# feiyuhuahuo/Yolact_minimal

Measured on AMD Instinct MI355X. Metric: img/s res101_coco 544x544 inference (bs=1/GPU, 4 requests in flight), higher is better.
Workload: dtype f32; 1 GPU; res101_coco 544x544 (the reference's "550-class" size) bs=1 inference: forward + nms + after_nms(480x640) per image, 4 independent bs=1 requests in flight on 4 HIP streams; global_batch=1, parallelism=replicas x1 (inference does not shard), weights=seeded random init, post_inputs=synthetic dense head outputs (17.8k candidates), requests_in_flight=4

## Files before the change

include/yolact_hip.h:

```cpp
#ifndef YOLACT_HIP_H
#define YOLACT_HIP_H

#include <stddef.h>
#include <stdint.h>

#ifdef __cplusplus
extern "C" {
#endif

#define YM_OK 0
#define YM_EINVAL (-1)
#define YM_ENOSPC (-2)
#define YM_ELAUNCH (-3)

#define YM_ACT_NONE 0
#define YM_ACT_RELU 1
#define YM_ACT_TANH 2
#define YM_ACT_GELU 3

typedef void* ym_stream_t;

int ym_abi_version(void);
const char* ym_last_error(void);

// ... 189 lines not shown
int ym_match_anchors_batch(const float* const* gt_boxes_cls, const int32_t* g, int B, const float* anchors, int N, float pos_thre,
                           float neg_thre, float* offsets, int64_t* conf, float* anchor_box, int64_t* anchor_gt, void* workspace,
                           size_t workspace_bytes, ym_stream_t s);

size_t ym_loss_workspace_bytes(int B, int N);
int ym_class_box_loss(const float* class_p, const float* box_p, const float* offsets, const int64_t* conf, int B, int N, int C,
                      float conf_alpha, float bbox_alpha, int neg_pos_ratio, float* dclass, float* dbox, int32_t* num_pos,
                      double* loss_c, double* loss_b, void* workspace, size_t workspace_bytes, ym_stream_t s);

int ym_select_positives(const int64_t* conf, const float* keys, int B, int N, int cap, const int32_t* num_pos, int64_t* idx,
                        ym_stream_t s);

int ym_gt_masks_downsample(const float* masks, int n, int H, int W, int out_h, int out_w, float* out, ym_stream_t s);

int ym_semantic_loss(const float* seg_nhwc, int P, int pitch, int num_classes, const float* gt_masks_ds, const int64_t* gt_cls,
                     int gt_cls_stride, int g, float coeff, float* dseg, double* loss_accum, ym_stream_t s);
int ym_semantic_loss_batch(const float* seg_nhwc, int B, int P, int pitch, int num_classes, const float* const* gt_masks_ds,
                           const int64_t* const* gt_cls, int gt_cls_stride, const int32_t* g, float coeff, float* dseg,
                           double* loss_accum, ym_stream_t s);

int ym_maxpool3x3s2_bwd(const float* x, const float* dy, float* dx, int B, int H, int W, int C, ym_stream_t s);
int ym_maxpool3x3s2_fwd_idx(const float* in, float* out, uint8_t* idx, int B, int H, int W, int C, ym_stream_t s);
int ym_maxpool3x3s2_bwd_idx(const uint8_t* idx, const float* dy, float* dx, int B, int H, int W, int C, ym_stream_t s);
int ym_bilinear2x_bwd(const float* dy, float* dx, int B, int H, int W, int C, int align_corners, ym_stream_t s);

int ym_sgd_step(float* param, const float* grad, float* momentum_buf, int64_t n, float lr, float momentum,
                float weight_decay, int first_step, ym_stream_t s);


int ym_maxpool3x3s2_fwd(const float* in, float* out, int B, int H, int W, int C, ym_stream_t s);
int ym_stem_conv_bn_relu_maxpool(const float* img_nchw, const float* w_packed, const float* scale, const float* shift, float* out,
                                 int B, int H, int W, int k_pad, ym_stream_t s);

int ym_bilinear2x_fwd(const float* in, float* out, int B, int H, int W, int C, int align_corners, ym_stream_t s);

int ym_softmax_rows(const float* in, float* out, int64_t rows, int C, ym_stream_t s);


int ym_layernorm(const float* x, const float* gamma, const float* beta, float eps, float* out, int64_t M, int C,
                 ym_stream_t s);

int ym_patch_merge_layernorm(const float* x, int B, int H, int W, int C, const float* gamma, const float* beta, float eps,
                             float* out, ym_stream_t s);

int ym_swin_window_attention(const float* qkv, const float* qkv_bias, const float* rel_bias_table, int B, int H, int W, int C,
                             int heads, int window, int shift, float* out, ym_stream_t s);


int ym_val_preprocess(const void* img_hwc_bgr, int is_uint8, int H, int W, int S, const float* mean_bgr,
                      const float* std_bgr, float* out_chw_rgb, ym_stream_t s);


typedef struct {
    int32_t num_anchors;
    int32_t num_classes;
    int32_t coef_dim;
    int32_t top_k;
    int32_t max_det;
    float score_thre;
    float iou_thre;
    float img_size;
} ym_nms_cfg;

size_t ym_nms_workspace_bytes(const ym_nms_cfg* cfg);

int ym_detect_fast_nms(const float* class_pred, const float* box_pred, const float* coef_pred,
// ... 124 lines not shown
```

yolact_minimal_amd/engine.py:

```python
import json
import os
import sys

import torch
import torch.nn as nn

from . import conv_launch, hip, plan_transfer
from .conv_plan import ConvPlan
from .hip import ACT_NONE, ACT_RELU, ACT_TANH, ACT_GELU


def _round_up(x, m):
    return (x + m - 1) // m * m


TUNED_PATH = os.environ.get('YM_TUNED_PATH', os.path.join(os.path.dirname(os.path.abspath(__file__)), 'tuned_gfx950.json'))
_tuned = None


def conv_mma():
    return int(os.environ.get('YM_CONV_MMA', '0') or 0)


def no_tuned():
# ... 135 lines not shown
        self._bind_params()
        self.out_hw = (ho, wo)
        self.flops = 2.0 * b * ho * wo * self.cout * self.kh * self.kw * self.cin
        self.sig = plan_transfer.forward_key(b * ho * wo, self.cout, cin, self.kh, self.stride, len(segs), residual is not None)
        self._shape = (b * ho * wo, self.cout, self.k_pad // 32, len(segs))
        self._resolve(conv_mma())
        return ho, wo

    def _resolve(self, mma, bound=None, pyramid=False):
        d = self.desc
        self.plan, self.mma, self.plan_source, self._hit = conv_launch.infer_plan(
            tuned_table(), self.sig, self._shape, _build_mode[0], mma, not self.stem and d.Cin % 32 == 0 and d.nlevels == 0, self.plan,
            no_tuned(), pyramid, bound)
        self.plan.apply(d)
        d.mma = self.mma

    def apply_mma(self, mma):
        self._resolve(mma, (self._hit, self.plan_source))


def _bind_pyramid(layer, pyr, batch, shapes, segs):
    rows, cin = pyr.shape
    assert cin == layer.cin_pad and layer.stride == 1 and layer.pad == layer.kh // 2 and len(shapes) <= 5
    assert rows == sum(batch * h * w for h, w in shapes)
    d = layer.desc = conv_launch.conv_desc(batch, shapes[0][0], shapes[0][1], cin, layer.cout, layer.kh, layer.kw, 1, layer.pad,
                                           shapes[0][0], shapes[0][1], layer.k_pad, segs, levels=shapes)
    d.inp = pyr.data_ptr()
    layer._bind_params()
    layer.out_hw = shapes[0]
    layer.flops = 2.0 * rows * layer.cout * layer.kh * layer.kw * layer.cin
    layer.sig = plan_transfer.forward_key(rows, layer.cout, cin, layer.kh, 1, len(segs), levels=len(shapes))
    layer._shape = (rows, layer.cout, layer.k_pad // 32, len(segs))
    layer._resolve(0, pyramid=True)


class InferEngine:
    def __init__(self, net, batch, height, width, device, use_graph=None, mode='latency'):
        self.net = net
        self.mode = mode
        self.device = device
        self.B, self.H, self.W = batch, height, width
        self.num_classes = net.cfg.num_classes
        self.coef_dim = net.coef_dim
        self.na = len(net.cfg.aspect_ratios)
        if use_graph is None:
            use_graph = os.environ.get('YM_GRAPH', '1') != '0'
        self.use_graph = use_graph
        self.graph = None
        self.ops = []
        self.op_stream = {}
        self.op_deps = {}
        self._producers = {}
        self._cur_stream = 0
        self._side_streams = {}
        self._events = {}
        self.use_branches = os.environ.get('YM_BRANCHES', '0') == '1'
        self.convs = []
        self.fused_stem = None
        self._img = None
        self._weights_epoch = -1
        self._bufs = []
        hip.lib()
        prev, _build_mode[0] = _build_mode[0], mode
        try:
            with torch.cuda.device(device):
                self._build()
                if autotune_on() and not no_tuned():
                    self._autotune_missing()
        finally:
            _build_mode[0] = prev

    def _autotune_missing(self):
        have = {c.sig for c in self.convs if c.plan_source == 'table'}
        todo = {c.sig for c in self.convs} - have
        if not todo:
            return
        rows = self.autotune(iters=10, skip=have)
        for c in self.convs:
            if c.sig in rows:
                c.plan_source, c._hit = 'autotuned', ConvPlan.from_row(rows[c.sig])
        record_rows(rows)

    def _buf(self, *shape):
        t = torch.empty(*shape, device=self.device, dtype=torch.float32)
        self._bufs.append(t)
        return t

    def _add_op(self, kind, arg, inputs, outputs):
        idx = len(self.ops)
        self.ops.append((kind, arg))
        sid = self._cur_stream if self.use_branches else 0
        self.op_stream[idx] = sid
        deps = []
        for t in inputs:
            if t is None:
                continue
            for j in self._producers.get(t.data_ptr(), ()):
                if self.op_stream[j] != sid and j not in deps:
                    deps.append(j)
        if deps:
            self.op_deps[idx] = deps
        for t in outputs:
            self._producers.setdefault(t.data_ptr(), []).append(idx)
        return idx

    def _conv(self, layer, x, out=None, residual=None, segs=None, seg_outputs=None):
        b, h, w, _ = x.shape
        ho = (h + 2 * layer.pad - layer.kh) // layer.stride + 1
        wo = (w + 2 * layer.pad - layer.kw) // layer.stride + 1
        if segs is None:
            if out is None:
                out = self._buf(b, ho, wo, layer.cout)
            segs = [(0, layer.cout, out.data_ptr(), ho * wo * layer.cout, layer.cout, layer.act)]
        layer.refresh()
        layer.bind(x, segs, residual)
        self.convs.append(layer)
        self._add_op('conv', layer, [x, residual], seg_outputs if seg_outputs is not None else [out])
        return out

    def _build_swin(self):
        net, B = self.net, self.B
        bb = net.backbone
        ws = bb.window_size
        assert self.H % 4 == 0 and self.W % 4 == 0
        pe = bb.patch_embed
        x = self._conv(_Conv('backbone.patch_embed.proj', pe.proj, act=ACT_NONE, stem=True), self.x_in)
        self._add_op('layernorm', (x, pe.norm, x), [x], [x])
        feats = []
        for li, layer in enumerate(bb.layers):
            _, h, w, c = x.shape
            heads = bb.heads[li]
            for bi, blk in enumerate(layer.blocks):
                p = f'backbone.layers.{li}.blocks.{bi}'
                n1 = self._buf(B, h, w, c)
                self._add_op('layernorm', (x, blk.norm1, n1), [x], [n1])
                qkv = self._conv(_Conv(p + '.attn.qkv', _LinearAsConv(blk.attn.qkv)), n1)
                att = self._buf(B, h, w, c)
                self._add_op('attn', (qkv, blk.attn, att, (B, h, w, c, heads, ws, blk.shift_size)), [qkv], [att])
                x = self._conv(_Conv(p + '.attn.proj', _LinearAsConv(blk.attn.proj)), att, residual=x)
                n2 = self._buf(B, h, w, c)
                self._add_op('layernorm', (x, blk.norm2, n2), [x], [n2])
                hid = self._conv(_Conv(p + '.mlp.fc1', _LinearAsConv(blk.mlp.fc1), act=ACT_GELU), n2)
                x = self._conv(_Conv(p + '.mlp.fc2', _LinearAsConv(blk.mlp.fc2)), hid, residual=x)
            if li in bb.out_norm_indices:
                f = self._buf(B, h, w, c)
                self._add_op('layernorm', (x, getattr(bb, f'norm{li}'), f), [x], [f])
                feats.append(f)
            if layer.downsample is not None:
                ho, wo = (h + 1) // 2, (w + 1) // 2
                merged = self._buf(B, ho, wo, 4 * c)
# ... 10 lines not shown
            c3, c4, c5 = self._build_swin()
        else:
            c3, c4, c5 = self._build_resnet()
        self._build_neck_and_heads(c3, c4, c5)

    def _build_resnet(self):
        net, B, H, W = self.net, self.B, self.H, self.W
        bb = net.backbone

        stem = _Conv('backbone.conv1', bb.conv1, bb.bn1, ACT_RELU, stem=True)
        conv1 = bb.conv1
        fusable = (conv1.out_channels == 64 and conv1.in_channels == 3 and tuple(conv1.kernel_size) == (7, 7) and
                   tuple(conv1.stride) == (2, 2) and tuple(conv1.padding) == (3, 3))
        if fusable and os.environ.get('YM_FUSED_STEM', '1') != '0':
            stem.refresh()
            ho, wo = (H + 6 - 7) // 2 + 1, (W + 6 - 7) // 2 + 1
            hp, wp = (ho + 2 - 3) // 2 + 1, (wo + 2 - 3) // 2 + 1
            stem.flops = 2.0 * B * ho * wo * stem.cout * stem.kh * stem.kw * stem.cin
            self.fused_stem = stem
            pooled = self._buf(B, hp, wp, 64)
            self._add_op('stem_pool', (stem, pooled), [], [pooled])
            x = pooled
        else:
            x = self._conv(stem, self.x_in)
            hp, wp = (x.shape[1] + 2 - 3) // 2 + 1, (x.shape[2] + 2 - 3) // 2 + 1
            pooled = self._buf(B, hp, wp, 64)
            self._add_op('maxpool', (x, pooled), [x], [pooled])
            x = pooled

        stage_outs = []
        for li, stage in enumerate(bb.layers):
            for bi, blk in enumerate(stage):
                p = f'backbone.layers.{li}.{bi}'
                y = self._conv(_Conv(p + '.conv1', blk.conv1, blk.bn1, ACT_RELU), x)
                y = self._conv(_Conv(p + '.conv2', blk.conv2, blk.bn2, ACT_RELU), y)
                if blk.downsample is not None:
                    skip = self._conv(_Conv(p + '.downsample', blk.downsample[0], blk.downsample[1], ACT_NONE), x)
                else:
                    skip = x
                x = self._conv(_Conv(p + '.conv3', blk.conv3, blk.bn3, ACT_RELU), y, residual=skip)
            stage_outs.append(x)
        return stage_outs[1:4]

    def _build_neck_and_heads(self, c3, c4, c5):
        net, B = self.net, self.B
        fpn = net.fpn
        p5_1 = self._conv(_Conv('fpn.lat_layers.2', fpn.lat_layers[2]), c5)
        u5 = self._buf(B, p5_1.shape[1] * 2, p5_1.shape[2] * 2, 256)
        self._add_op('bilinear', (p5_1, u5, False), [p5_1], [u5])
        assert u5.shape[1:3] == c4.shape[1:3], 'img_size must be divisible by 32 (reference config.py:75)'
        p4_1 = self._conv(_Conv('fpn.lat_layers.1', fpn.lat_layers[1]), c4, residual=u5)
        u4 = self._buf(B, p4_1.shape[1] * 2, p4_1.shape[2] * 2, 256)
        self._add_op('bilinear', (p4_1, u4, False), [p4_1], [u4])
        p3_1 = self._conv(_Conv('fpn.lat_layers.0', fpn.lat_layers[0]), c3, residual=u4)
        pyr_env = os.environ.get('YM_PYRAMID_HEAD', 'auto')
        pyramid = pyr_env == '1' or (pyr_env == 'auto' and B <= 2)
        h5, w5 = p5_1.shape[1:3]
        shapes = [tuple(p3_1.shape[1:3]), tuple(p4_1.shape[1:3]), (h5, w5), ((h5 + 1) // 2, (w5 + 1) // 2),
                  (((h5 + 1) // 2 + 1) // 2, ((w5 + 1) // 2 + 1) // 2)]
        rows = [B * h * w for h, w in shapes]
        pyr = self._buf(sum(rows), 256)
        views, r0 = [], 0
        for (h, w), n in zip(shapes, rows):
            views.append(pyr[r0:r0 + n].view(B, h, w, 256))
            r0 += n
        self._cur_stream = 1
        p5 = self._conv(_Conv('fpn.pred_layers.2', fpn.pred_layers[2][0], act=ACT_RELU), p5_1, out=views[2])
        p6 = self._conv(_Conv('fpn.downsample_layers.0', fpn.downsample_layers[0][0], act=ACT_RELU), p5, out=views[3])
        p7 = self._conv(_Conv('fpn.downsample_layers.1', fpn.downsample_layers[1][0], act=ACT_RELU), p6, out=views[4])
        self._cur_stream = 2
        p4 = self._conv(_Conv('fpn.pred_layers.1', fpn.pred_layers[1][0], act=ACT_RELU), p4_1, out=views[1])
        self._cur_stream = 0
        p3 = self._conv(_Conv('fpn.pred_layers.0', fpn.pred_layers[0][0], act=ACT_RELU), p3_1, out=views[0])
# ... 37 lines not shown
            self.convs.append(fused)
            self._add_op('conv', fused, [xh], [self.class_logits, self.box_pred, self.coef_pred])
        off = 0
        for li, lv in enumerate(levels if not pyramid else []):
            self._cur_stream = level_stream[li]
            xh = self._conv(_Conv(f'prediction_layers.upfeature@P{li + 3}', hd.upfeature[0], act=ACT_RELU), lv)
            fused = _Conv(f'prediction_layers.conf|bbox|coef@P{li + 3}', [hd.conf_layer, hd.bbox_layer, hd.coef_layer[0]])
            es = 4
            segs = [
                (0, c_conf, self.class_logits.data_ptr() + off * nc * es, n_total * nc, c_conf, ACT_NONE),
                (c_conf, c_conf + c_box, self.box_pred.data_ptr() + off * 4 * es, n_total * 4, c_box, ACT_NONE),
                (c_conf + c_box, c_conf + c_box + c_coef, self.coef_pred.data_ptr() + off * cd * es, n_total * cd,
                 c_coef, ACT_TANH),
            ]
            self._conv(fused, xh, segs=segs, seg_outputs=[self.class_logits, self.box_pred, self.coef_pred])
            off += lv.shape[1] * lv.shape[2] * na
        self._cur_stream = 0
        self._add_op('softmax', (self.class_logits, self.class_pred), [self.class_logits], [self.class_pred])

        self._alloc_workspaces()
        self.total_flops = sum(c.flops for c in self.convs) + (self.fused_stem.flops if self.fused_stem is not None else 0.0)
        self._weights_epoch = self.net._weights_epoch

    def _alloc_workspaces(self):
        sids = {self.op_stream.get(i, 0) for i, (kind, _) in enumerate(self.ops) if kind == 'conv'} | {0}
        fused = os.environ.get('YM_FUSED_SPLITK', '1') != '0'
        oldc = getattr(self, 'counters', {})
        self.counters = {sid: oldc[sid] if sid in oldc else torch.zeros(hip.TILE_COUNTERS, device=self.device, dtype=torch.int32)
                         for sid in sids}
        need = {sid: 256 for sid in sids}
        for i, (kind, arg) in enumerate(self.ops):
            if kind == 'conv':
                sid = self.op_stream.get(i, 0)
                arg.desc.tile_counters = self.counters[sid].data_ptr() if fused else None
                if not fused:
                    arg.desc.tail_tiles, arg.desc.tail_ksplit = 0, 0
                nb = hip.conv_workspace_bytes(arg.desc)
                need[sid] = max(need[sid], nb)
        need[0] = max(need.values())
        old = getattr(self, 'workspaces', {})
        self.workspaces = {sid: (old[sid] if sid in old and old[sid].numel() >= nb else
                                 torch.empty(nb, device=self.device, dtype=torch.uint8)) for sid, nb in need.items()}
        self.workspace = self.workspaces[0]

    def refresh_weights(self):
        for c in self.convs:
            c.refresh()
        if self.fused_stem is not None:
            self.fused_stem.refresh()
        self._weights_epoch = self.net._weights_epoch
        self.graph = None

    def retune(self):
        for c in self.convs:
            c.plan.apply(c.desc)
            c.desc.mma = c.mma
        self._alloc_workspaces()
        self.graph = None

    def set_mma(self, mma):
        prev, _build_mode[0] = _build_mode[0], self.mode
        try:
            for c in self.convs:
                c.apply_mma(mma)
        finally:
            _build_mode[0] = prev
        self.retune()

    def autotune(self, iters=10, verbose=False, mma=0, concurrent=False, skip=(), cus=256):
        results = {}
        self.autotune_detail = {}
# ... 106 lines not shown
                        if kwv == 8 and tm * tn == 4096:
                            continue
                        if waves * kwv > 65536:
                            continue
                        cands.append(ConvPlan(tm, tn, 1, kwv))
                if d.Cin % 32 == 0 and d.nlevels == 0:
                    for tm, tn in ((32, 32), (64, 32), (32, 64)):
                        for kwv in (1, 2, 4):
                            if kwv <= nkt:
                                wave_cands.append(ConvPlan(tm, tn, 1, kwv, 22))
                                wave_cands += [ConvPlan(tm, tn, 1, kwv, 22, grid_wgs=wpb) for wpb in (1, 2) if wpb >= kwv and kwv < 4]
                    tiles32 = -(-M // 32) * -(-d.Cout // 32)
                    if cus < tiles32 <= hip.TILE_COUNTERS and d.nseg == 1 and d.tile_counters:
                        wave_cands += [ConvPlan(32, 32, 1, 4, 22, tiles32 % cus or cus, ts) for ts in (4, 6, 8) if ts * 2 <= nkt]
            if mma:
                cands = sorted({p._replace(stages=st) for p in cands for st in ((0, 3) if not p.wave else (0,))})
            best, p = base, ConvPlan()
            for cand in cands + ([] if mma else wave_cands):
                t = time_cfg(c, cand)
                if t is not None and t < best * 0.98:
                    best, p = t, cand
            c.plan = seen[c.sig] = p
            c.mma = mma if (mma and not p.wave) else 0
            results[c.sig + (f'_mma{mma}' if mma else '')] = p.to_row()
            self.autotune_detail[c.sig + (f'_mma{mma}' if mma else '')] = (round(best, 2), round(base, 2))
            if verbose:
                print(f'{c.sig:44s} default {base:8.1f} us -> {p.to_row()} {best:8.1f} us', flush=True)
        del big_ws
        self.retune()
        return results

    def _launch_one(self, kind, arg, ws):
        if kind == 'conv':
            hip.conv2d_fwd(arg.desc, ws)
        elif kind == 'maxpool':
            hip.maxpool3x3s2(arg[0], arg[1])
        elif kind == 'stem_pool':
            hip.stem_conv_bn_relu_maxpool(self._img, arg[0].weight, arg[0].scale, arg[0].shift, arg[1])
        elif kind == 'bilinear':
            hip.bilinear2x(arg[0], arg[1], arg[2])
        elif kind == 'softmax':
            hip.softmax_rows(arg[0], arg[1])
        elif kind == 'layernorm':
            hip.layernorm(arg[0], arg[1].weight.detach(), arg[1].bias.detach(), arg[1].eps, arg[2])
        elif kind == 'merge_ln':
            hip.patch_merge_layernorm(arg[0], arg[1].weight.detach(), arg[1].bias.detach(), arg[1].eps, arg[2])
        elif kind == 'attn':
            qkv, attn, out, (b, h, w, c, heads, win, shift) = arg
            hip.swin_window_attention(qkv, attn.qkv.bias.detach(), attn.relative_position_bias_table.detach(), b, h, w, c,
                                      heads, win, shift, out)

    def _launch_all(self, img):
        if self.fused_stem is None:
            hip.nchw_to_nhwc4(img, self.x_in)
        self._img = img
        main = torch.cuda.current_stream()
        needs_event = {j for deps in self.op_deps.values() for j in deps}
        used = set()
        for i, (kind, arg) in enumerate(self.ops):
            sid = self.op_stream.get(i, 0)
            if sid == 0:
                st = main
            else:
                st = self._side_streams.get(sid)
                if st is None:
                    st = self._side_streams[sid] = torch.cuda.Stream(device=self.device)
                used.add(sid)
# ... 57 lines not shown
```

yolact_minimal_amd/hip.py:

```python
import ctypes
import os

import torch

_PKG = os.path.dirname(os.path.abspath(__file__))
LIB_PATH = os.environ.get('YM_LIB_PATH') or os.path.join(_PKG, 'libyolact_hip.so')

ACT_NONE, ACT_RELU, ACT_TANH, ACT_GELU = 0, 1, 2, 3
DRAW_HIDE_MASK, DRAW_HIDE_BBOX, DRAW_HIDE_SCORE, DRAW_REAL_TIME = 1, 2, 4, 8
DRAW_FONT_ADVANCE, DRAW_FONT_HEIGHT, DRAW_NAME_STRIDE, DRAW_LABEL_MAX, DRAW_MAX_DET = 12, 14, 40, 44, 512
EVAL_MAX_DET, EVAL_MAX_THRESHOLDS, EVAL_AP_ROWS_PER_PASS = 1024, 16, 1024
COCO_MAX_GT, COCO_AREAS, COCO_WORDS_PER_ROW, COCO_ROWS_PER_PASS = 512, 4, 8, 1024

ABI_SYMBOLS = (
    'ym_abi_version', 'ym_last_error', 'ym_nchw_to_nhwc4', 'ym_pack_conv_weight', 'ym_fold_bn',
    'ym_sizeof_conv_desc', 'ym_conv2d_workspace_bytes', 'ym_conv2d_tile_counters', 'ym_conv2d_fwd', 'ym_maxpool3x3s2_fwd', 'ym_stem_conv_bn_relu_maxpool', 'ym_bilinear2x_fwd',
    'ym_softmax_rows', 'ym_nms_workspace_bytes', 'ym_detect_fast_nms', 'ym_detect_greedy_nms',
    'ym_greedy_nms_workspace_bytes', 'ym_greedy_nms', 'ym_mask_assemble', 'ym_mask_resize_binarize',
    'ym_boxes_to_pixels', 'ym_expf_cr', 'ym_nms_batch_workspace_bytes', 'ym_detect_fast_nms_batch', 'ym_after_nms_batch_workspace_bytes',
    'ym_after_nms_batch', 'ym_head_grad_gather', 'ym_scatter3',
    'ym_greedy_nms_batch_workspace_bytes', 'ym_detect_greedy_nms_batch',
    'ym_pack_conv_weight_dgrad', 'ym_pack_conv_weights_batch', 'ym_conv2d_wgrad_workspace_bytes', 'ym_conv2d_wgrad', 'ym_conv2d_wgrad_slabs', 'ym_wgrad_reduce_batch', 'ym_bn_train_fwd',
    'ym_val_preprocess', 'ym_layernorm', 'ym_patch_merge_layernorm', 'ym_swin_window_attention',
    'ym_mask_loss_workspace_bytes', 'ym_mask_loss_fwd_bwd', 'ym_mask_loss_batch_workspace_bytes', 'ym_mask_loss_batch',
    'ym_mask_iou_workspace_bytes', 'ym_mask_iou', 'ym_box_iou', 'ym_match_detections', 'ym_rle_encode', 'ym_ann_to_mask_workspace_bytes', 'ym_poly_to_mask', 'ym_runs_to_mask', 'ym_train_aug_image', 'ym_train_aug_masks',
    'ym_layernorm_bwd_workspace_bytes', 'ym_layernorm_bwd', 'ym_patch_merge_layernorm_bwd', 'ym_gelu_fwd', 'ym_gelu_bwd',
    'ym_swin_window_attention_bwd', 'ym_adamw_step', 'ym_drop_path_add', 'ym_drop_path_bwd', 'ym_select_positives',
    'ym_match_anchors', 'ym_match_anchors_batch', 'ym_loss_workspace_bytes', 'ym_class_box_loss', 'ym_semantic_loss',
    'ym_semantic_loss_batch', 'ym_gt_masks_downsample',
    'ym_draw_workspace_bytes', 'ym_draw_detections_batch', 'ym_draw_cutout_objects',
    'ym_after_nms_batch_packed', 'ym_pack_masks', 'ym_unpack_masks', 'ym_mask_iou_packed_workspace_bytes', 'ym_mask_iou_packed',
    'ym_rle_encode_packed', 'ym_draw_detections_batch_packed', 'ym_draw_cutout_objects_packed',
    'ym_bn_train_bwd_workspace_bytes', 'ym_bn_train_bwd', 'ym_bn_train_bwd_apply', 'ym_act_bias_bwd', 'ym_conv2d_fuses_bn_stats', 'ym_bn_train_fwd_stats', 'ym_maxpool3x3s2_bwd', 'ym_maxpool3x3s2_fwd_idx', 'ym_maxpool3x3s2_bwd_idx', 'ym_bilinear2x_bwd', 'ym_sgd_step',
    'ym_conv2d_bn_partial_rows', 'ym_conv2d_effective_plan', 'ym_bn_partials_finish', 'ym_unordered_sum_launches', 'ym_bn_train_fwd_workspace_bytes',
    'ym_eval_match_log', 'ym_eval_ap_workspace_bytes', 'ym_eval_ap',
    'ym_coco_iou_box', 'ym_coco_iou_mask_packed', 'ym_coco_match_log', 'ym_coco_accumulate_workspace_bytes', 'ym_coco_accumulate',
    'ym_after_nms_ragged_workspace_bytes', 'ym_after_nms_ragged', 'ym_after_nms_ragged_packed',
)


class ConvSeg(ctypes.Structure):
    _fields_ = [('n_begin', ctypes.c_int), ('n_end', ctypes.c_int), ('out', ctypes.c_void_p),
                ('batch_stride', ctypes.c_int64), ('pitch', ctypes.c_int32), ('act', ctypes.c_int32)]


class ConvDesc(ctypes.Structure):
    _fields_ = [('inp', ctypes.c_void_p), ('weight', ctypes.c_void_p), ('scale', ctypes.c_void_p),
                ('shift', ctypes.c_void_p), ('residual', ctypes.c_void_p),
                ('B', ctypes.c_int32), ('H', ctypes.c_int32), ('W', ctypes.c_int32), ('Cin', ctypes.c_int32),
# ... 55 lines not shown
    _fields_ = [('img_h', ctypes.c_int32), ('img_w', ctypes.c_int32), ('offset', ctypes.c_int64)]


RAGGED_MAX_IMAGES = 32
RAGGED_ALIGN_BYTES = 256

_lib = None


def lib():
    global _lib
    if _lib is None:
        if not os.path.exists(LIB_PATH):
            raise RuntimeError(
                f'{LIB_PATH} is missing: build it with `python -c "import __graft_entry__ as g; g.build()"` '
                f'(or `make -C yolact_minimal_amd/csrc`). yolact_minimal_amd has no non-HIP fallback.')
        L = ctypes.CDLL(LIB_PATH)
        vp, i32, i64, f32, sz = ctypes.c_void_p, ctypes.c_int, ctypes.c_int64, ctypes.c_float, ctypes.c_size_t
        L.ym_abi_version.restype = ctypes.c_int
        L.ym_last_error.restype = ctypes.c_char_p
        L.ym_nchw_to_nhwc4.argtypes = [vp, vp, i32, i32, i32, i32, vp]
        L.ym_pack_conv_weight.argtypes = [vp, vp, i32, i32, i32, i32, i32, i32, vp]
        L.ym_fold_bn.argtypes = [vp, vp, vp, vp, f32, vp, vp, i32, vp]
        L.ym_sizeof_conv_desc.restype = sz
        if L.ym_sizeof_conv_desc() != ctypes.sizeof(ConvDesc):
            raise RuntimeError(f'libyolact_hip.so was built from a different ym_conv_desc ({L.ym_sizeof_conv_desc()} B) than '
                               f'yolact_minimal_amd/hip.py mirrors ({ctypes.sizeof(ConvDesc)} B): rebuild the library')
        L.ym_conv2d_workspace_bytes.argtypes = [ctypes.POINTER(ConvDesc)]
        L.ym_conv2d_workspace_bytes.restype = sz
        L.ym_conv2d_fwd.argtypes = [ctypes.POINTER(ConvDesc), vp, sz, vp]
        L.ym_conv2d_tile_counters.argtypes = [ctypes.POINTER(ConvDesc)]
        L.ym_maxpool3x3s2_fwd.argtypes = [vp, vp, i32, i32, i32, i32, vp]
        L.ym_stem_conv_bn_relu_maxpool.argtypes = [vp, vp, vp, vp, vp, i32, i32, i32, i32, vp]
        L.ym_bilinear2x_fwd.argtypes = [vp, vp, i32, i32, i32, i32, i32, vp]
        L.ym_softmax_rows.argtypes = [vp, vp, i64, i32, vp]
        L.ym_nms_workspace_bytes.argtypes = [ctypes.POINTER(NmsCfg)]
        L.ym_nms_workspace_bytes.restype = sz
        nms_args = [vp, vp, vp, vp, ctypes.POINTER(NmsCfg), vp, vp, vp, vp, vp, vp, sz, vp]
        L.ym_detect_fast_nms.argtypes = nms_args
        L.ym_detect_greedy_nms.argtypes = nms_args
        L.ym_greedy_nms_workspace_bytes.argtypes = [i32]
        L.ym_greedy_nms_workspace_bytes.restype = sz
        L.ym_greedy_nms.argtypes = [vp, i32, f32, vp, vp, vp, sz, vp]
        L.ym_mask_assemble.argtypes = [vp, vp, vp, i32, i32, i32, i32, i32, vp, vp]
        L.ym_mask_resize_binarize.argtypes = [vp, i32, i32, i32, i32, i32, vp, vp]
        L.ym_boxes_to_pixels.argtypes = [vp, vp, i32, f32, vp]
        L.ym_expf_cr.argtypes = [vp, vp, i64, vp]
        L.ym_nms_batch_workspace_bytes.argtypes = [ctypes.POINTER(NmsCfg), i32]
        L.ym_nms_batch_workspace_bytes.restype = sz
        L.ym_detect_fast_nms_batch.argtypes = [vp, vp, vp, vp, ctypes.POINTER(NmsCfg), i32, vp, vp, vp, vp, vp, vp, sz, vp]
        L.ym_greedy_nms_batch_workspace_bytes.argtypes = L.ym_nms_batch_workspace_bytes.argtypes
        L.ym_greedy_nms_batch_workspace_bytes.restype = sz
        L.ym_detect_greedy_nms_batch.argtypes = L.ym_detect_fast_nms_batch.argtypes
        L.ym_after_nms_batch_workspace_bytes.argtypes = [i32, i32, i32, i32, i32]
        L.ym_after_nms_batch_workspace_bytes.restype = sz
        L.ym_after_nms_batch.argtypes = [vp, vp, vp, vp, i32, i32, i32, i32, i32, i32, i32, i32, vp, vp, vp, sz, vp]
        L.ym_head_grad_gather.argtypes = [vp, vp, vp, vp, i32, i32, i32, i32, i32, i32, vp, vp, i32, vp, vp, vp]
        L.ym_scatter3.argtypes = [vp, vp, i32, vp, i32, vp, i32, i32, vp]
        L.ym_pack_conv_weight_dgrad.argtypes = [vp, vp, i32, i32, i32, i32, i32, vp]
        L.ym_pack_conv_weights_batch.argtypes = [vp, i32, i32, vp]
        L.ym_conv2d_wgrad_workspace_bytes.argtypes = [ctypes.POINTER(WgradDesc)]
        L.ym_conv2d_wgrad_workspace_bytes.restype = sz
        L.ym_conv2d_wgrad.argtypes = [ctypes.POINTER(WgradDesc), vp, sz, vp]
        L.ym_conv2d_wgrad_slabs.argtypes = [ctypes.POINTER(WgradDesc), vp, sz, ctypes.POINTER(WgradReduceItem), vp]
        L.ym_wgrad_reduce_batch.argtypes = [vp, i32, ctypes.c_uint32, vp]
        L.ym_bn_train_fwd.argtypes = [vp, i64, i32, vp, vp, f32, f32, vp, vp, vp, i32, vp, vp, vp, vp, sz, vp]
# ... 147 lines not shown
    return n


def conv_effective_plan(desc):
    from .conv_plan import ConvPlan
    row = (ctypes.c_int32 * 8)()
    check(lib().ym_conv2d_effective_plan(ctypes.byref(desc), ctypes.byref(row)), 'ym_conv2d_effective_plan')
    return ConvPlan(*row)


TILE_COUNTERS = 16384


def conv2d_fwd(desc, workspace=None):
    counters = desc.tile_counters
    if counters and lib().ym_conv2d_tile_counters(ctypes.byref(desc)) > TILE_COUNTERS:
        desc.tile_counters = None
    ws_ptr = ctypes.c_void_p(workspace.data_ptr()) if workspace is not None else None
    ws_bytes = workspace.numel() * workspace.element_size() if workspace is not None else 0
    try:
        check(lib().ym_conv2d_fwd(ctypes.byref(desc), ws_ptr, ws_bytes, stream_ptr()), 'ym_conv2d_fwd')
    finally:
        desc.tile_counters = counters


def stem_conv_bn_relu_maxpool(img, w_packed, scale, shift, out):
    b, c, h, w = img.shape
    if c != 3 or tuple(w_packed.shape) != (64, 224):
        raise RuntimeError(f'stem: expects a 3-channel image and a [64, 224] packed filter, got {tuple(img.shape)} / {tuple(w_packed.shape)}')
    check(lib().ym_stem_conv_bn_relu_maxpool(ptr(img), ptr(w_packed), ptr(scale), ptr(shift), ptr(out), b, h, w, w_packed.shape[1],
                                             stream_ptr()), 'ym_stem_conv_bn_relu_maxpool')


def maxpool3x3s2(x, out):
    b, h, w, c = x.shape
    check(lib().ym_maxpool3x3s2_fwd(ptr(x), ptr(out), b, h, w, c, stream_ptr()), 'ym_maxpool3x3s2_fwd')


def bilinear2x(x, out, align_corners):
    b, h, w, c = x.shape
    check(lib().ym_bilinear2x_fwd(ptr(x), ptr(out), b, h, w, c, int(bool(align_corners)), stream_ptr()),
          'ym_bilinear2x_fwd')


def softmax_rows(x, out):
    c = x.shape[-1]
    rows = x.numel() // c
    check(lib().ym_softmax_rows(ptr(x), ptr(out), rows, c, stream_ptr()), 'ym_softmax_rows')


def layernorm(x, gamma, beta, eps, out):
    c = x.shape[-1]
    check(lib().ym_layernorm(ptr(x), ptr(gamma), ptr(beta), float(eps), ptr(out), x.numel() // c, c, stream_ptr()), 'ym_layernorm')


def patch_merge_layernorm(x, gamma, beta, eps, out):
    b, h, w, c = x.shape
    check(lib().ym_patch_merge_layernorm(ptr(x), b, h, w, c, ptr(gamma), ptr(beta), float(eps), ptr(out), stream_ptr()),
          'ym_patch_merge_layernorm')


def swin_window_attention(qkv, qkv_bias, table, b, h, w, c, heads, window, shift, out):
    check(lib().ym_swin_window_attention(ptr(qkv), ptr(qkv_bias), ptr(table), b, h, w, c, heads, window, shift, ptr(out),
                                         stream_ptr()), 'ym_swin_window_attention')


# ... 29 lines not shown
```

Baseline: 513.2 img/s.

## Fuse ResNet stage-1 bottleneck convs into one tiled MFMA kernel

Adds a single HIP kernel that runs conv1 (1x1), conv2 (3x3) and conv3 (1x1) of a 64-mid bottleneck, plus the optional downsample and residual add, on an 8x8 spatial tile held in LDS. It recomputes the 1x1 conv over the halo so intermediates never go to global memory. The engine swaps eligible blocks (Cin 64/256, stage 1, under a tile-count limit) for this op, enabled by default. The aim is to cut launch count and DRAM traffic for intermediates, at the cost of halo recompute and high LDS use per workgroup.

```diff
diff --git a/include/yolact_hip.h b/include/yolact_hip.h
--- a/include/yolact_hip.h
+++ b/include/yolact_hip.h
@@ -245,6 +245,12 @@
 int ym_stem_conv_bn_relu_maxpool(const float* img_nchw, const float* w_packed, const float* scale, const float* shift, float* out,
                                  int B, int H, int W, int k_pad, ym_stream_t s);
 
+int ym_bottleneck_fwd(const float* x, const float* w1, const float* scale1, const float* shift1,
+                      const float* w2, const float* scale2, const float* shift2,
+                      const float* w3, const float* scale3, const float* shift3,
+                      const float* wd, const float* scaled, const float* shiftd,
+                      float* out, int B, int H, int W, int Cin, ym_stream_t s);
+
 int ym_bilinear2x_fwd(const float* in, float* out, int B, int H, int W, int C, int align_corners, ym_stream_t s);
 
 int ym_softmax_rows(const float* in, float* out, int64_t rows, int C, ym_stream_t s);
diff --git a/yolact_minimal_amd/csrc/conv_bottleneck.hip b/yolact_minimal_amd/csrc/conv_bottleneck.hip
--- /dev/null
+++ b/yolact_minimal_amd/csrc/conv_bottleneck.hip
@@ -0,0 +1,329 @@
+#include "conv_common.h"
+
+using namespace ymk;
+
+namespace {
+
+constexpr int TH = 8, TW = 8;
+constexpr int HP = TW + 2;
+constexpr int HROWS = (TH + 2) * HP;
+constexpr int M1 = 128;
+constexpr int MID = 64, COUT = 256;
+constexpr int T1_F = M1 * MID;
+constexpr int T2_F = TH * TW * MID;
+constexpr int A_STAGE = M1 * BK, W_STAGE = 64 * BK;
+constexpr int P1_STAGE = A_STAGE + W_STAGE;
+constexpr int NS1 = 3, D1 = NS1 - 1;
+constexpr int NSW = 3, DW = NSW - 1;
+constexpr int NT2 = 9 * MID / BK;
+constexpr int CP = COUT + 4;
+constexpr int LDS_F = NS1 * P1_STAGE;
+constexpr size_t BNK_LDS = (size_t)LDS_F * sizeof(float);
+static_assert(T1_F + T2_F + NSW * W_STAGE <= LDS_F, "phase 2 / 3 fit into phase 1's footprint");
+static_assert(T1_F + T2_F >= 2 * P1_STAGE, "the filter ring of phase 2 starts in phase 1's last stage, clear of t1 and t2");
+static_assert(TH * TW * CP <= LDS_F, "the staged output tile");
+static_assert(HROWS <= M1 && TH * TW == 64 && TW == 8, "tile shape");
+static_assert(BNK_LDS <= 80 * 1024, "two workgroups per CU");
+
+struct BnkP {
+    const float *x, *w1, *w2, *w3, *wd;
+    const float *s1, *b1, *s2, *b2, *s3, *b3, *sd, *bd;
+    float* out;
+    int B, H, W, Cin;
+    FastDiv fd_tiles, fd_tx;
+    unsigned x_bytes, w1_bytes;
+};
+
+constexpr int WAIT_ALL = 0x0070;
+constexpr int WAIT_P1 = 0x0070 | (6 * (D1 - 1));
+static_assert(6 * (D1 - 1) < 16 && 2 * (DW - 1) < 16, "vmcnt field");
+constexpr int WAIT_RING = 0x0070 | (2 * (DW - 1));
+
+__device__ __forceinline__ int t_off(int row, int chunk) { return row * MID + ((chunk ^ (row & 15)) << 2); }
+
+template <bool DS>
+__global__ __launch_bounds__(256) void k_bottleneck(const BnkP p) {
+    typedef __attribute__((address_space(3))) void* lds_ptr;
+    extern __shared__ __attribute__((aligned(16))) float smem[];
+    float* P1 = smem;
+    float* T1 = smem;
+    float* T2 = smem + T1_F;
+    float* WR = smem + T1_F + T2_F;
+    float* CS = smem;
+
+    const int tid = threadIdx.x;
+    const int lane = tid & 63, wave = __builtin_amdgcn_readfirstlane(tid >> 6);
+    const int frag_row = lane & 31, khalf = lane >> 5;
+    const int wm = wave >> 1, wn = wave & 1;
+
+    unsigned ub, urem, uty, utx;
+    p.fd_tiles.divmod((unsigned)ym_xcd_remap(blockIdx.x, gridDim.x), ub, urem);
+    p.fd_tx.divmod(urem, uty, utx);
+    const int b = (int)ub, y0 = (int)uty * TH, x0 = (int)utx * TW;
+    const int H = p.H, W = p.W, Cin = p.Cin;
+
+    const __amdgpu_buffer_rsrc_t rs_x = __builtin_amdgcn_make_buffer_rsrc((void*)p.x, 0, p.x_bytes, 0x00020000);
+    const __amdgpu_buffer_rsrc_t rs_w1 = __builtin_amdgcn_make_buffer_rsrc((void*)p.w1, 0, p.w1_bytes, 0x00020000);
+    const __amdgpu_buffer_rsrc_t rs_w2 = __builtin_amdgcn_make_buffer_rsrc((void*)p.w2, 0, MID * 9 * MID * 4, 0x00020000);
+    const __amdgpu_buffer_rsrc_t rs_w3 = __builtin_amdgcn_make_buffer_rsrc((void*)p.w3, 0, COUT * MID * 4, 0x00020000);
+    const __amdgpu_buffer_rsrc_t rs_wd = __builtin_amdgcn_make_buffer_rsrc((void*)(DS ? p.wd : p.w3), 0, COUT * MID * 4, 0x00020000);
+
+    const int c4 = (tid & 7) ^ ((tid >> 4) & 7);
+    const int rbase = tid >> 3;
+    unsigned a_off[4];
+#pragma unroll
+    for (int i = 0; i < 4; ++i) {
+        const int row = rbase + 32 * i;
+        const int hy = row / HP, hx = row - hy * HP;
+        const int gy = y0 - 1 + hy, gx = x0 - 1 + hx;
+        const bool ok = row < HROWS && (unsigned)gy < (unsigned)H && (unsigned)gx < (unsigned)W;
+        a_off[i] = ok ? (unsigned)((((b * H + gy) * W + gx) * Cin + c4 * 4) * 4) : OOB;
+    }
+    unsigned w1_off[2], w2_off[2], w3_off[2];
+#pragma unroll
+    for (int i = 0; i < 2; ++i) {
+        const int n = rbase + 32 * i;
+        w1_off[i] = (unsigned)((n * Cin + c4 * 4) * 4);
+        w2_off[i] = (unsigned)((n * 9 * MID + c4 * 4) * 4);
+        w3_off[i] = (unsigned)((n * MID + c4 * 4) * 4);
+    }
+    int goff[4];
+#pragma unroll
+    for (int g = 0; g < 4; ++g) goff[g] = ((2 * g + khalf) ^ ((frag_row >> 1) & 7)) * 4;
+
+    const float sc1[2] = {p.s1[frag_row], p.s1[32 + frag_row]}, sh1[2] = {p.b1[frag_row], p.b1[32 + frag_row]};
+    const int nk1 = Cin / BK;
+    auto p1_issue = [&](int kt, int buf) __attribute__((always_inline)) {
+        float* a = P1 + buf * P1_STAGE + 8 * wave * BK;
+        float* w = a + A_STAGE;
+#pragma unroll
+        for (int i = 0; i < 4; ++i) __builtin_amdgcn_raw_ptr_buffer_load_lds(rs_x, (lds_ptr)(a + 32 * i * BK), 16, (int)a_off[i], kt * BK * 4, 0, 0);
+#pragma unroll
+        for (int i = 0; i < 2; ++i) __builtin_amdgcn_raw_ptr_buffer_load_lds(rs_w1, (lds_ptr)(w + 32 * i * BK), 16, (int)w1_off[i], kt * BK * 4, 0, 0);
+    };
+    f32x16 acc1[2];
+#pragma unroll
+    for (int j = 0; j < 2; ++j)
+#pragma unroll
+        for (int r = 0; r < 16; ++r) acc1[j][r] = 0.f;
+#pragma unroll
+    for (int d = 0; d < D1; ++d)
+        if (d < nk1) p1_issue(d, d);
+    if (nk1 > D1 - 1) __builtin_amdgcn_s_waitcnt(WAIT_P1); else __builtin_amdgcn_s_waitcnt(WAIT_ALL);
+    __builtin_amdgcn_s_barrier();
+#pragma unroll 1
+    for (int kt = 0; kt < nk1; ++kt) {
+        const int buf = kt % NS1;
+        const bool more = kt + D1 < nk1;
+        if (more) p1_issue(kt + D1, (kt + D1) % NS1);
+        const float* a = P1 + buf * P1_STAGE + (wave * 32 + frag_row) * BK;
+        const float* w = P1 + buf * P1_STAGE + A_STAGE + frag_row * BK;
+#pragma unroll
+        for (int g = 0; g < 4; ++g) {
+            const f32x4 fa = *reinterpret_cast<const f32x4*>(a + goff[g]);
+            const f32x4 fb0 = *reinterpret_cast<const f32x4*>(w + goff[g]);
+            const f32x4 fb1 = *reinterpret_cast<const f32x4*>(w + 32 * BK + goff[g]);
+#pragma unroll
+            for (int s = 0; s < 4; ++s) {
+                acc1[0] = __builtin_amdgcn_mfma_f32_32x32x2f32(fa[s], fb0[s], acc1[0], 0, 0, 0);
+                acc1[1] = __builtin_amdgcn_mfma_f32_32x32x2f32(fa[s], fb1[s], acc1[1], 0, 0, 0);
+            }
+        }
+        if (more) __builtin_amdgcn_s_waitcnt(WAIT_P1); else __builtin_amdgcn_s_waitcnt(WAIT_ALL);
+        __builtin_amdgcn_s_barrier();
+    }
+
+    constexpr int TPN = DS ? 4 : 2;
+    constexpr int NT3 = 4 * TPN;
+    auto w_issue = [&](int q) __attribute__((always_inline)) {
+        float* dst = WR + (q % NSW) * W_STAGE + 8 * wave * BK;
+        if (q < NT2) {
+#pragma unroll
+            for (int i = 0; i < 2; ++i) __builtin_amdgcn_raw_ptr_buffer_load_lds(rs_w2, (lds_ptr)(dst + 32 * i * BK), 16, (int)w2_off[i], q * BK * 4, 0, 0);
+        } else {
+            const int q3 = q - NT2, nb = q3 / TPN, j = q3 - nb * TPN;
+            const bool live = q3 < NT3;
+            const int soff = live ? (nb * 64 * MID + (j & 1) * BK) * 4 : 0;
+            if (DS && j >= 2) {
+#pragma unroll
+                for (int i = 0; i < 2; ++i) __builtin_amdgcn_raw_ptr_buffer_load_lds(rs_wd, (lds_ptr)(dst + 32 * i * BK), 16, (int)(live ? w3_off[i] : OOB), soff, 0, 0);
+            } else {
+#pragma unroll
+                for (int i = 0; i < 2; ++i) __builtin_amdgcn_raw_ptr_buffer_load_lds(rs_w3, (lds_ptr)(dst + 32 * i * BK), 16, (int)(live ? w3_off[i] : OOB), soff, 0, 0);
+            }
+        }
+    };
+    const int m_frag = wm * 32 + frag_row;
+    f32x4 xa[DS ? 8 : 1];
+    if constexpr (DS) {
+        const int gy = y0 + (m_frag >> 3), gx = x0 + (m_frag & 7);
+        const bool ok = gy < H && gx < W;
+        const unsigned base = ok ? (unsigned)((((b * H + gy) * W + gx) * Cin + khalf * 4) * 4) : OOB;
+#pragma unroll
+        for (int u = 0; u < 8; ++u) xa[u] = buf_ld16_s(rs_x, base, (u * 8) * 4);
+    }
+#pragma unroll
+    for (int d = 0; d < DW; ++d) w_issue(d);
+
+#pragma unroll
+    for (int r = 0; r < 16; ++r) {
+        const int row = wave * 32 + 4 * khalf + (r & 3) + 8 * (r >> 2);
+        const int hy = row / HP, hx = row - hy * HP;
+        const int gy = y0 - 1 + hy, gx = x0 - 1 + hx;
+        const bool ok = row < HROWS && (unsigned)gy < (unsigned)H && (unsigned)gx < (unsigned)W;
+#pragma unroll
+        for (int j = 0; j < 2; ++j) {
+            const int ch = j * 32 + frag_row;
+            float v = __builtin_fmaf(acc1[j][r], sc1[j], sh1[j]);
+            v = v < 0.f ? 0.f : v;
+            T1[t_off(row, ch >> 2) + (ch & 3)] = ok ? v : 0.f;
+        }
+    }
+    __builtin_amdgcn_s_waitcnt(WAIT_RING);
+    __syncthreads();
+
+    const int ch2 = wn * 32 + frag_row;
+    const float sc2 = p.s2[ch2], sh2 = p.b2[ch2];
+    const int hr0 = (m_frag >> 3) * HP + (m_frag & 7);
+    f32x16 acc_e, acc_o;
+#pragma unroll
+    for (int r = 0; r < 16; ++r) { acc_e[r] = 0.f; acc_o[r] = 0.f; }
+    const int bfrag = (wn * 32 + frag_row) * BK;
+#pragma unroll 1
+    for (int q = 0; q < NT2; ++q) {
+        w_issue(q + DW);
+        const int tap = q >> 1, kh = tap / 3, kw = tap - 3 * kh;
+        const int hr = hr0 + kh * HP + kw, kc = (q & 1) * 8;
+        const float* w = WR + (q % NSW) * W_STAGE + bfrag;
+#pragma unroll
+        for (int g = 0; g < 4; ++g) {
+            const f32x4 fa = *reinterpret_cast<const f32x4*>(T1 + t_off(hr, kc + 2 * g + khalf));
+            const f32x4 fb = *reinterpret_cast<const f32x4*>(w + goff[g]);
+            acc_e = __builtin_amdgcn_mfma_f32_32x32x2f32(fa[0], fb[0], acc_e, 0, 0, 0);
+            acc_o = __builtin_amdgcn_mfma_f32_32x32x2f32(fa[1], fb[1], acc_o, 0, 0, 0);
+            acc_e = __builtin_amdgcn_mfma_f32_32x32x2f32(fa[2], fb[2], acc_e, 0, 0, 0);
+            acc_o = __builtin_amdgcn_mfma_f32_32x32x2f32(fa[3], fb[3], acc_o, 0, 0, 0);
+        }
+        __builtin_amdgcn_s_waitcnt(WAIT_RING);
+        __builtin_amdgcn_s_barrier();
+    }
+    acc_e += acc_o;
+#pragma unroll
+    for (int r = 0; r < 16; ++r) {
+        const int m = wm * 32 + 4 * khalf + (r & 3) + 8 * (r >> 2);
+        float v = __builtin_fmaf(acc_e[r], sc2, sh2);
+        v = v < 0.f ? 0.f : v;
+        T2[t_off(m, ch2 >> 2) + (ch2 & 3)] = v;
+    }
+    __builtin_amdgcn_s_waitcnt(WAIT_ALL);
+    __syncthreads();
+
+    f32x4 a3[8];
+#pragma unroll
+    for (int u = 0; u < 8; ++u) a3[u] = *reinterpret_cast<const f32x4*>(T2 + t_off(m_frag, 2 * u + khalf));
+    f32x16 acc3[4], accd[DS ? 4 : 1];
+#pragma unroll
+    for (int nb = 0; nb < 4; ++nb)
+#pragma unroll
+        for (int r = 0; r < 16; ++r) { acc3[nb][r] = 0.f; if (DS) accd[DS ? nb : 0][r] = 0.f; }
+#pragma unroll
+    for (int nb = 0; nb < 4; ++nb) {
+#pragma unroll
+        for (int j = 0; j < TPN; ++j) {
+            const int q = NT2 + nb * TPN + j;
+            w_issue(q + DW);
+            const float* w = WR + (q % NSW) * W_STAGE + bfrag;
+#pragma unroll
+            for (int g = 0; g < 4; ++g) {
+                const f32x4 fb = *reinterpret_cast<const f32x4*>(w + goff[g]);
+                const f32x4 fa = j < 2 ? a3[(j & 1) * 4 + g] : xa[DS ? (j & 1) * 4 + g : 0];
+#pragma unroll
+                for (int s = 0; s < 4; ++s) {
+                    if (j < 2) acc3[nb] = __builtin_amdgcn_mfma_f32_32x32x2f32(fa[s], fb[s], acc3[nb], 0, 0, 0);
+                    else accd[DS ? nb : 0] = __builtin_amdgcn_mfma_f32_32x32x2f32(fa[s], fb[s], accd[DS ? nb : 0], 0, 0, 0);
+                }
+            }
+            __builtin_amdgcn_s_waitcnt(WAIT_RING);
+            __builtin_amdgcn_s_barrier();
+        }
+    }
+    __builtin_amdgcn_s_waitcnt(WAIT_ALL);
+    __syncthreads();
+
+    const int col4 = tid & 63, row0 = tid >> 6;
+#pragma unroll
+    for (int nb = 0; nb < 4; ++nb) {
+        const int ch3 = nb * 64 + wn * 32 + frag_row;
+        const float sc3 = p.s3[ch3], sh3 = p.b3[ch3];
+        float scd = 0.f, shd = 0.f;
+        if constexpr (DS) { scd = p.sd[ch3]; shd = p.bd[ch3]; }
+#pragma unroll
+        for (int r = 0; r < 16; ++r) {
+            const int m = wm * 32 + 4 * khalf + (r & 3) + 8 * (r >> 2);
+            float v = __builtin_fmaf(acc3[nb][r], sc3, sh3);
+            if constexpr (DS) v += __builtin_fmaf(accd[DS ? nb : 0][r], scd, shd);
+            CS[m * CP + ch3] = v;
+        }
+    }
+    f32x4 res[DS ? 1 : 16];
+    if constexpr (!DS) {
+#pragma unroll
+        for (int k = 0; k < 16; ++k) {
+            const int row = row0 + 4 * k;
+            const int gy = y0 + (row >> 3), gx = x0 + (row & 7);
+            res[k] = buf_ld16(rs_x, (gy < H && gx < W) ? (unsigned)((((b * H + gy) * W + gx) * COUT + col4 * 4) * 4) : OOB);
+        }
+    }
+    __syncthreads();
+#pragma unroll
+    for (int k = 0; k < 16; ++k) {
+        const int row = row0 + 4 * k;
+        const int gy = y0 + (row >> 3), gx = x0 + (row & 7);
+        f32x4 v = *reinterpret_cast<const f32x4*>(CS + row * CP + col4 * 4);
+        if constexpr (!DS) v += res[k];
+#pragma unroll
+        for (int e = 0; e < 4; ++e) v[e] = v[e] < 0.f ? 0.f : v[e];
+        if (gy < H && gx < W) *reinterpret_cast<f32x4*>(p.out + (((size_t)b * H + gy) * W + gx) * COUT + col4 * 4) = v;
+    }
+}
+
+}
+
+extern "C" int ym_bottleneck_fwd(const float* x, const float* w1, const float* scale1, const float* shift1,
+                                 const float* w2, const float* scale2, const float* shift2,
+                                 const float* w3, const float* scale3, const float* shift3,
+                                 const float* wd, const float* scaled, const float* shiftd,
+                                 float* out, int B, int H, int W, int Cin, ym_stream_t s) {
+    YM_REQUIRE(x && w1 && scale1 && shift1 && w2 && scale2 && shift2 && w3 && scale3 && shift3 && out, "bottleneck: null argument");
+    YM_REQUIRE(B > 0 && H > 0 && W > 0, "bottleneck: bad shape %d x %d x %d", B, H, W);
+    const bool ds = wd != nullptr;
+    YM_REQUIRE(!ds || (scaled && shiftd), "bottleneck: the downsample conv needs its scale and shift");
+    YM_REQUIRE(ds ? Cin == 64 : Cin == 256, "bottleneck: Cin must be 256 (identity skip) or 64 (with the downsample conv), got %d%s", Cin,
+               ds ? " with a downsample conv" : "");
+    YM_REQUIRE(x != out, "bottleneck: in-place is not supported (tiles read each other's halo)");
+    const uintptr_t al = (uintptr_t)x | (uintptr_t)w1 | (uintptr_t)w2 | (uintptr_t)w3 | (uintptr_t)wd | (uintptr_t)out;
+    YM_REQUIRE((al & 15) == 0, "bottleneck: tensors must be 16-byte aligned");
+    const long long xb = (long long)B * H * W * Cin * 4;
+    YM_REQUIRE(xb < (1ll << 31) && (long long)B * H * W * COUT * 4 < (1ll << 33), "bottleneck: input too large for 32-bit offsets");
+    const int tiles_y = ym_cdiv(H, TH), tiles_x = ym_cdiv(W, TW);
+    const long long grid = (long long)B * tiles_y * tiles_x;
+    YM_REQUIRE(grid < (1ll << 31), "bottleneck: grid too large");
+    BnkP p = {};
+    p.x = x; p.w1 = w1; p.w2 = w2; p.w3 = w3; p.wd = wd;
+    p.s1 = scale1; p.b1 = shift1; p.s2 = scale2; p.b2 = shift2; p.s3 = scale3; p.b3 = shift3; p.sd = scaled; p.bd = shiftd;
+    p.out = out;
+    p.B = B; p.H = H; p.W = W; p.Cin = Cin;
+    p.fd_tiles = FastDiv::make((unsigned)(tiles_y * tiles_x));
+    p.fd_tx = FastDiv::make((unsigned)tiles_x);
+    p.x_bytes = (unsigned)xb;
+    p.w1_bytes = (unsigned)(MID * Cin * 4);
+    static YmLdsAttr attr_id = {}, attr_ds = {};
+    if (ds) {
+        if (int rc = ym_ensure_dyn_lds(attr_ds, reinterpret_cast<const void*>(k_bottleneck<true>), BNK_LDS, "bottleneck_fwd")) return rc;
+        hipLaunchKernelGGL(k_bottleneck<true>, dim3((unsigned)grid), dim3(256), BNK_LDS, (hipStream_t)s, p);
+    } else {
+        if (int rc = ym_ensure_dyn_lds(attr_id, reinterpret_cast<const void*>(k_bottleneck<false>), BNK_LDS, "bottleneck_fwd")) return rc;
+        hipLaunchKernelGGL(k_bottleneck<false>, dim3((unsigned)grid), dim3(256), BNK_LDS, (hipStream_t)s, p);
+    }
+    return ym_check_launch("bottleneck_fwd");
+}
diff --git a/yolact_minimal_amd/engine.py b/yolact_minimal_amd/engine.py
--- a/yolact_minimal_amd/engine.py
+++ b/yolact_minimal_amd/engine.py
@@ -191,6 +191,60 @@
     layer.sig = plan_transfer.forward_key(rows, layer.cout, cin, layer.kh, 1, len(segs), levels=len(shapes))
     layer._shape = (rows, layer.cout, layer.k_pad // 32, len(segs))
     layer._resolve(0, pyramid=True)
+
+
+def fused_bottleneck_on():
+    return os.environ.get('YM_FUSED_BOTTLENECK', '1') != '0'
+
+
+class _FusedBottleneck:
+    fused = True
+    plan_source = 'fused'
+    mma = 0
+
+    def __init__(self, name, conv1, conv2, conv3, down, x, out):
+        self.name = name
+        self.conv1, self.conv2, self.conv3, self.down = conv1, conv2, conv3, down
+        self.members = [conv1, conv2] + ([down] if down is not None else []) + [conv3]
+        self.x, self.out = x, out
+        b, h, w, cin = x.shape
+        self.flops = sum(m.flops for m in self.members)
+        self.sig = f'bottleneck_M{b * h * w}_C{cin}_d{int(down is not None)}'
+
+    @staticmethod
+    def eligible(blk):
+        c1, c2, c3 = blk.conv1, blk.conv2, blk.conv3
+        ok = (tuple(c1.kernel_size) == (1, 1) and tuple(c1.stride) == (1, 1) and tuple(c1.padding) == (0, 0) and c1.out_channels == 64 and
+              tuple(c2.kernel_size) == (3, 3) and tuple(c2.stride) == (1, 1) and tuple(c2.padding) == (1, 1) and
+              tuple(getattr(c2, 'dilation', (1, 1))) == (1, 1) and c2.in_channels == 64 and c2.out_channels == 64 and
+              tuple(c3.kernel_size) == (1, 1) and tuple(c3.stride) == (1, 1) and c3.in_channels == 64 and c3.out_channels == 256 and
+              all(c.bias is None and getattr(c, 'groups', 1) == 1 for c in (c1, c2, c3)))
+        if not ok:
+            return False
+        if blk.downsample is None:
+            return c1.in_channels == 256
+        d = blk.downsample[0]
+        return (c1.in_channels == 64 and tuple(d.kernel_size) == (1, 1) and tuple(d.stride) == (1, 1) and tuple(d.padding) == (0, 0) and
+                d.in_channels == 64 and d.out_channels == 256 and d.bias is None)
+
+    RESIDENT_TILES = 512
+
+    @staticmethod
+    def worth(b, h, w, down):
+        return down or b * (-(-h // 8)) * (-(-w // 8)) <= _FusedBottleneck.RESIDENT_TILES
+
+    @property
+    def active(self):
+        return all(m.mma == 0 for m in self.members)
+
+    def launch(self, ws):
+        if not self.active:
+            for m in self.members:
+                hip.conv2d_fwd(m.desc, ws)
+            return
+        parts = [(m.weight, m.scale, m.shift) for m in (self.conv1, self.conv2, self.conv3)]
+        down = (self.down.weight, self.down.scale, self.down.shift) if self.down is not None else None
+        hip.bottleneck_fwd(self.x, parts[0], parts[1], parts[2], self.out, down)
 
 
 class InferEngine:
@@ -215,6 +269,7 @@
         self._events = {}
         self.use_branches = os.environ.get('YM_BRANCHES', '0') == '1'
         self.convs = []
+        self.fused_blocks = []
         self.fused_stem = None
         self._img = None
         self._weights_epoch = -1
@@ -263,7 +318,7 @@
             self._producers.setdefault(t.data_ptr(), []).append(idx)
         return idx
 
-    def _conv(self, layer, x, out=None, residual=None, segs=None, seg_outputs=None):
+    def _conv(self, layer, x, out=None, residual=None, segs=None, seg_outputs=None, add_op=True):
         b, h, w, _ = x.shape
         ho = (h + 2 * layer.pad - layer.kh) // layer.stride + 1
         wo = (w + 2 * layer.pad - layer.kw) // layer.stride + 1
@@ -274,7 +329,8 @@
         layer.refresh()
         layer.bind(x, segs, residual)
         self.convs.append(layer)
-        self._add_op('conv', layer, [x, residual], seg_outputs if seg_outputs is not None else [out])
+        if add_op:
+            self._add_op('conv', layer, [x, residual], seg_outputs if seg_outputs is not None else [out])
         return out
 
     def _build_swin(self):
@@ -351,13 +407,25 @@
         for li, stage in enumerate(bb.layers):
             for bi, blk in enumerate(stage):
                 p = f'backbone.layers.{li}.{bi}'
-                y = self._conv(_Conv(p + '.conv1', blk.conv1, blk.bn1, ACT_RELU), x)
-                y = self._conv(_Conv(p + '.conv2', blk.conv2, blk.bn2, ACT_RELU), y)
+                fuse = (fused_bottleneck_on() and _FusedBottleneck.eligible(blk) and
+                        _FusedBottleneck.worth(B, x.shape[1], x.shape[2], blk.downsample is not None))
+                c1 = _Conv(p + '.conv1', blk.conv1, blk.bn1, ACT_RELU)
+                c2 = _Conv(p + '.conv2', blk.conv2, blk.bn2, ACT_RELU)
+                c3 = _Conv(p + '.conv3', blk.conv3, blk.bn3, ACT_RELU)
+                cd = None
+                y = self._conv(c1, x, add_op=not fuse)
+                y = self._conv(c2, y, add_op=not fuse)
                 if blk.downsample is not None:
-                    skip = self._conv(_Conv(p + '.downsample', blk.downsample[0], blk.downsample[1], ACT_NONE), x)
+                    cd = _Conv(p + '.downsample', blk.downsample[0], blk.downsample[1], ACT_NONE)
+                    skip = self._conv(cd, x, add_op=not fuse)
                 else:
                     skip = x
-                x = self._conv(_Conv(p + '.conv3', blk.conv3, blk.bn3, ACT_RELU), y, residual=skip)
+                out = self._conv(c3, y, residual=skip, add_op=not fuse)
+                if fuse:
+                    fb = _FusedBottleneck(p, c1, c2, c3, cd, x, out)
+                    self.fused_blocks.append(fb)
+                    self._add_op('conv', fb, [x], [out])
+                x = out
             stage_outs.append(x)
         return stage_outs[1:4]
 
@@ -461,11 +529,12 @@
         for i, (kind, arg) in enumerate(self.ops):
             if kind == 'conv':
                 sid = self.op_stream.get(i, 0)
-                arg.desc.tile_counters = self.counters[sid].data_ptr() if fused else None
-                if not fused:
-                    arg.desc.tail_tiles, arg.desc.tail_ksplit = 0, 0
-                nb = hip.conv_workspace_bytes(arg.desc)
-                need[sid] = max(need[sid], nb)
+                for c in getattr(arg, 'members', (arg,)):
+                    c.desc.tile_counters = self.counters[sid].data_ptr() if fused else None
+                    if not fused:
+                        c.desc.tail_tiles, c.desc.tail_ksplit = 0, 0
+                    nb = hip.conv_workspace_bytes(c.desc)
+                    need[sid] = max(need[sid], nb)
         need[0] = max(need.values())
         old = getattr(self, 'workspaces', {})
         self.workspaces = {sid: (old[sid] if sid in old and old[sid].numel() >= nb else
@@ -638,7 +707,10 @@
 
     def _launch_one(self, kind, arg, ws):
         if kind == 'conv':
-            hip.conv2d_fwd(arg.desc, ws)
+            if getattr(arg, 'fused', False):
+                arg.launch(ws)
+            else:
+                hip.conv2d_fwd(arg.desc, ws)
         elif kind == 'maxpool':
             hip.maxpool3x3s2(arg[0], arg[1])
         elif kind == 'stem_pool':
diff --git a/yolact_minimal_amd/hip.py b/yolact_minimal_amd/hip.py
--- a/yolact_minimal_amd/hip.py
+++ b/yolact_minimal_amd/hip.py
@@ -14,7 +14,7 @@
 
 ABI_SYMBOLS = (
     'ym_abi_version', 'ym_last_error', 'ym_nchw_to_nhwc4', 'ym_pack_conv_weight', 'ym_fold_bn',
-    'ym_sizeof_conv_desc', 'ym_conv2d_workspace_bytes', 'ym_conv2d_tile_counters', 'ym_conv2d_fwd', 'ym_maxpool3x3s2_fwd', 'ym_stem_conv_bn_relu_maxpool', 'ym_bilinear2x_fwd',
+    'ym_sizeof_conv_desc', 'ym_conv2d_workspace_bytes', 'ym_conv2d_tile_counters', 'ym_conv2d_fwd', 'ym_maxpool3x3s2_fwd', 'ym_stem_conv_bn_relu_maxpool', 'ym_bottleneck_fwd', 'ym_bilinear2x_fwd',
     'ym_softmax_rows', 'ym_nms_workspace_bytes', 'ym_detect_fast_nms', 'ym_detect_greedy_nms',
     'ym_greedy_nms_workspace_bytes', 'ym_greedy_nms', 'ym_mask_assemble', 'ym_mask_resize_binarize',
     'ym_boxes_to_pixels', 'ym_expf_cr', 'ym_nms_batch_workspace_bytes', 'ym_detect_fast_nms_batch', 'ym_after_nms_batch_workspace_bytes',
@@ -136,6 +136,7 @@
         L.ym_conv2d_tile_counters.argtypes = [ctypes.POINTER(ConvDesc)]
         L.ym_maxpool3x3s2_fwd.argtypes = [vp, vp, i32, i32, i32, i32, vp]
         L.ym_stem_conv_bn_relu_maxpool.argtypes = [vp, vp, vp, vp, vp, i32, i32, i32, i32, vp]
+        L.ym_bottleneck_fwd.argtypes = [vp] * 14 + [i32, i32, i32, i32, vp]
         L.ym_bilinear2x_fwd.argtypes = [vp, vp, i32, i32, i32, i32, i32, vp]
         L.ym_softmax_rows.argtypes = [vp, vp, i64, i32, vp]
         L.ym_nms_workspace_bytes.argtypes = [ctypes.POINTER(NmsCfg)]
@@ -349,6 +350,16 @@
                                              stream_ptr()), 'ym_stem_conv_bn_relu_maxpool')
 
 
+def bottleneck_fwd(x, conv1, conv2, conv3, out, down=None):
+    b, h, w, cin = x.shape
+    shapes = [tuple(t[0].shape) for t in (conv1, conv2, conv3)] + ([tuple(down[0].shape)] if down is not None else [])
+    if shapes[:3] != [(64, cin), (64, 576), (256, 64)] or shapes[3:] not in ([], [(256, 64)]) or tuple(out.shape) != (b, h, w, 256):
+        raise RuntimeError(f'bottleneck: packed filters {shapes} / output {tuple(out.shape)} do not fit input {tuple(x.shape)}')
+    dn = down if down is not None else (None, None, None)
+    args = [ptr(x)] + [ptr(t) for c in (conv1, conv2, conv3, dn) for t in c] + [ptr(out)]
+    check(lib().ym_bottleneck_fwd(*args, b, h, w, cin, stream_ptr()), 'ym_bottleneck_fwd')
+
+
 def maxpool3x3s2(x, out):
     b, h, w, c = x.shape
     check(lib().ym_maxpool3x3s2_fwd(ptr(x), ptr(out), b, h, w, c, stream_ptr()), 'ym_maxpool3x3s2_fwd')
```

After: 520.6 img/s (median of 6 runs). +1.4%, better.
